# 87003697/DynamiCrafter

Hardware: AMD Instinct MI355X
Metric: frames/sec (and denoising-step ms), 16f@576x1024, DDIM 50 (higher is better)
Workload: dtype bf16; 1 GPU; inference_1024_v1.0.yaml: 1 clip/GPU, 16 frames, latent 72x128, DDIM 50 uniform_trailing eta=1, CFG 7.5 batched (cond+uncond), guidance_rescale 0.7, v-param+ZTSNR+dynamic rescale, hipGraph-captured step; clips_per_gpu=1, parallelism=dp1 over 1 distinct clips (no data-path collective), conditioning=local (1 rank), outputs_finite=True

## Files before the change

### dynamicrafter_amd/_hip.py

```python
import ctypes as C
import os
import threading

_HERE = os.path.dirname(os.path.abspath(__file__))
LIB_PATH = os.environ.get("DC_HIP_LIB") or os.path.join(_HERE, "csrc", "libdcrafter_hip.so")

DC_GEMM_OUT_F32 = 1
DC_GEMM_GEGLU = 2
DC_GEMM_GELU = 4


class DcGemmParams(C.Structure):
    _fields_ = [
        ("A", C.c_void_p), ("W", C.c_void_p), ("C", C.c_void_p), ("bias", C.c_void_p),
        ("rowvec", C.c_void_p), ("residual", C.c_void_p),
        ("lda", C.c_int), ("ldc", C.c_int), ("ldr", C.c_int), ("rowvec_ld", C.c_int),
        ("rows_per_vec", C.c_int),
        ("M", C.c_int), ("N", C.c_int), ("K", C.c_int), ("n_pad", C.c_int),
        ("mode", C.c_int), ("Cin", C.c_int),
        ("IH", C.c_int), ("IW", C.c_int), ("OH", C.c_int), ("OW", C.c_int),
        ("stride", C.c_int), ("pad", C.c_int), ("ups", C.c_int),
        ("T", C.c_int), ("HW", C.c_int),
        ("flags", C.c_int), ("alpha", C.c_float),
        ("workspace", C.c_void_p), ("workspace_bytes", C.c_longlong),
# ... 49 lines not shown
        ("step_index", C.c_void_p), ("index", C.c_int), ("weight_type", C.c_int), ("x0_param", C.c_int),
        ("e_nchw", C.c_int), ("cfg_scale", C.c_float), ("guidance_rescale", C.c_float),
        ("beta2", C.c_float), ("eps", C.c_float), ("one_minus_beta1", C.c_float), ("one_minus_beta2", C.c_float),
        ("decay", C.c_float), ("grad_scale", C.c_float), ("noise_step_stride", C.c_int64), ("loss", C.c_void_p),
    ]


_P, _I, _F, _L = C.c_void_p, C.c_int, C.c_float, C.c_int64
SIGNATURES = {
    "dc_gemm_conv": (_I, [C.POINTER(DcGemmParams), _P]),
    "dc_gemm_workspace_bytes": (_L, []),
    "dc_gemm_last_variant": (C.c_char_p, []),
    "dc_gemm_set_plan": (_I, [_I]),
    "dc_groupnorm": (_I, [_P, _I, _P, _I, _P, _P, _I, _I, _I, _I, _F, _I, _P, _P]),
    "dc_groupnorm_workspace_bytes": (_L, [_I, _I, _I]),
    "dc_layernorm": (_I, [_P, _I, _P, _I, _P, _P, _I, _I, _F, _P]),
    "dc_flash_attn_d64": (_I, [_P, _P, _P, _P, _I, _I, _I, _I, _I, _I, _I, _I, _L, _L, _F, _I, _F, _P]),
    "dc_ff_geglu_fused320": (_I, [_P, _I, _P, _P, _F, _P, _P, _P, _P, _P, _I, _P, _I, _I, _P]),
    "dc_ff_geglu_proj_fused320": (_I, [_P, _I, _P, _P, _F, _P, _P, _P, _P, _P, _P, _P, _I, _P, _I, _I, _P]),
    "dc_ln_linear": (_I, [_P, _I, _I, _P, _P, _F, _P, _P, _P, _I, _I, _I, _P]),
    "dc_ln_qkv_temporal_attn320": (_I, [_P, _I, _P, _P, _F, _P, _P, _I, _I, _I, _I, _F, _P]),
    "dc_ln_qkv_temporal_attn640": (_I, [_P, _I, _P, _P, _F, _P, _P, _I, _I, _I, _I, _F, _P]),
    "dc_gn_silu_tconv3": (_I, [_P, _I, _I, _P, _P, _P, _I, _P, _P, _P, _I, _P, _I, _I, _I, _I, _I, _P]),
    "dc_groupnorm_stats": (_I, [_P, _I, _I, _I, _I, _I, _F, _P, _P, _P]),
    "dc_gn_linear": (_I, [_P, _I, _I, _P, _P, _P, _I, _I, _P, _P, _P, _I, _I, _I, _P]),
    "dc_flash_attn_set_mode": (_I, [_I, _F]),
    "dc_linear_residual": (_I, [_P, _I, _I, _P, _P, _P, _I, _P, _I, _I, _I, _P]),
    "dc_cross_attn_dual_d64": (_I, [_P, _P, _P, _P, _P, _P, _I, _I, _I, _I, _I, _I, _I, _I, _L, _L, _F, _F, _P]),
    "dc_temporal_attn_d64": (_I, [_P, _I, _P, _I, _I, _I, _I, _I, _F, _P]),
    "dc_gemv_small": (_I, [_P, _I, _P, _P, _P, _I, _I, _I, _I, _I, _I, _I, _P]),
    "dc_timestep_embedding": (_I, [_P, _P, _I, _P, _I, _I, _F, _P]),
    "dc_pack_latent": (_I, [_P, _P, _P, _I, _I, _I, _I, _I, _I, _I, _P]),
    "dc_pack_latent_windows": (_I, [_P, _P, _P, _P, _P] + [_I] * 13 + [_P]),
    "dc_window_merge": (_I, [_P, _I, _P, _I, _P, _P, _P] + [_I] * 12 + [_P]),
    "dc_nchw_to_rows": (_I, [_P, _P, _I, _I, _I, _I, _F, _P]),
    "dc_rows_to_nchw": (_I, [_P, _I, _I, _P, _I, _I, _I, _F, _P]),
    "dc_im2col3x3_c8": (_I, [_P, _I, _P, _I, _I, _I, _I, _P]),
    "dc_copy2d": (_I, [_P, _I, _P, _I, _I, _I, _P]),
    "dc_build_context": (_I, [_P, _P, _I, _I, _I, _I, _I, _P]),
    "dc_softmax_rows": (_I, [_P, _I, _P, _I, _I, _I, _P]),
    "dc_transpose": (_I, [_P, _I, _P, _I, _I, _I, _P]),
    "dc_add_rows": (_I, [_P, _I, _P, _I, _P, _I, _I, _I, _P]),
    "dc_vae_sample": (_I, [_P, _I, _P, _P, _I, _I, _I, _F, _P]),
    "dc_ddim_step": (_I, [C.POINTER(DcDdimParams), _P, _P, _P, _I, _P, _P, _P, _P, _I, _I, _I, _P, _P]),
    "dc_ddim_invert_step": (_I, [C.POINTER(DcInvertParams), _P, _P, _P, _I, _P, _P, _P, _I, _I, _I, _P, _P]),
    "dc_dpmpp_step": (_I, [C.POINTER(DcDpmParams), _P, _P, _P, _I, _P, _P, _P, _P, _I, _I, _I, _P, _P]),
# ... 92 lines not shown
```

### dynamicrafter_amd/csrc/dc_common.h

```cpp
#pragma once
#include <hip/hip_runtime.h>
#include <stdint.h>
#include <atomic>

typedef uint16_t bf16_t;

typedef __attribute__((ext_vector_type(8))) short bf16x8_t;
typedef __attribute__((ext_vector_type(4))) short bf16x4_t;
typedef __attribute__((ext_vector_type(16))) float f32x16_t;
typedef __attribute__((ext_vector_type(4))) float f32x4_t;
typedef __attribute__((ext_vector_type(4))) unsigned int u32x4_t;

#define DC_WAVE 64

__device__ __forceinline__ float bf2f(bf16_t v) {
    return __uint_as_float(((uint32_t)v) << 16);
}

typedef __attribute__((ext_vector_type(2))) float f32x2_t;
typedef __attribute__((ext_vector_type(2))) __bf16 bf16x2_hw_t;

__device__ __forceinline__ uint32_t pack_bf2(float lo, float hi) {
    const f32x2_t v = {lo, hi};
    return __builtin_bit_cast(uint32_t, __builtin_convertvector(v, bf16x2_hw_t));
// ... 67 lines not shown
    return v;
}
__device__ __forceinline__ float wave_max(float v) {
#pragma unroll
    for (int o = 32; o > 0; o >>= 1) v = fmaxf(v, __shfl_xor(v, o, 64));
    return v;
}

__device__ __forceinline__ int xcd_remap(int bid, int nwg) {
    const int q = nwg >> 3, r = nwg & 7;
    const int xcd = bid & 7, idx = bid >> 3;
    const int base = (xcd < r) ? xcd * (q + 1) : r * (q + 1) + (xcd - r) * q;
    return base + idx;
}

void dc_note_variant(const char* name);

int dc_gemm_plan_now();

int dc_flash_pipe_launch(const bf16_t* q, const bf16_t* k, const bf16_t* v, bf16_t* o, int ldq, int ldk, int ldv, int ldo,
                         int batch, int heads, int Lq, int Lk, int64_t q_bstride, int64_t kv_bstride, float c,
                         hipStream_t stream);

int* dc_error_word_device();
#define DC_ERRW_GEMM_PIPE 1
#define DC_ERRW_FLASH_RING 2
#define DC_ERRW_GEMM_PP 4

struct DcLdsOnce {
    std::atomic<unsigned long long> done{0};
    int ensure(const void* fn, int bytes) {
        int dev = 0;
        hipError_t e = hipGetDevice(&dev);
        if (e != hipSuccess) return (int)e;
        const bool tracked = dev >= 0 && dev < 64;
        if (tracked && (done.load(std::memory_order_acquire) >> dev & 1ull)) return 0;
        e = hipFuncSetAttribute(fn, hipFuncAttributeMaxDynamicSharedMemorySize, bytes);
        if (e != hipSuccess) return (int)e;
        if (tracked) done.fetch_or(1ull << dev, std::memory_order_release);
        return 0;
    }
};

#define DC_CHECK_LAUNCH() do { hipError_t e__ = hipGetLastError(); if (e__ != hipSuccess) return (int)e__; } while (0)
```

### dynamicrafter_amd/csrc/ff_fused.hip

```cpp
#include "attn_parts.h"
#include "dc_common.h"
#include "dcrafter_hip.h"
#include "lds_stage.h"
#include <stdint.h>
#include <type_traits>

namespace {

constexpr int FD = 320;
constexpr int FM = 4 * FD;
constexpr int FCH = 32;
constexpr int FNCH = FM / FCH;
constexpr int FBM = 128;
constexpr int W1_STAGE = 64 * FD * 2;
constexpr int W2_STAGE = FD * FCH * 2;
constexpr int W2_RING = 3;
constexpr int FF_LDS = 2 * W1_STAGE + W2_RING * W2_STAGE + 4 * 2048 + 2 * FM * 4;
static_assert(FF_LDS <= 160 * 1024, "LDS");

#ifdef DC_FF_STAMPS
__device__ unsigned long long g_ff_stamps[8];
#define FF_STAMP(i) do { asm volatile("s_waitcnt lgkmcnt(0)" ::: "memory"); const unsigned long long t__ = __builtin_readcyclecounter(); \
                         st_acc[i] += t__ - st_last; st_last = t__; } while (0)
#else
// ... 833 lines not shown
        {
            const int rrow = lane >> 3, rc = lane & 7;
#pragma unroll
            for (int t = 0; t < 4; ++t) {
                const int r = t * 8 + rrow;
                const u32x4_t d = *reinterpret_cast<const u32x4_t*>(vpatch + lds_off128(r, rc));
                *reinterpret_cast<u32x4_t*>(p.O + grow(r) * p.ldo + 64 * h + rc * 8) = d;
            }
        }
    }
}


struct TcParams {
    const bf16_t* X; int ldx;
    const bf16_t* W;
    const float* bias;
    const bf16_t* R; int ldr;
    bf16_t* O; int ldo;
    const float* gn_g; const float* gn_b; const float2* gn_stats; int gn_groups;
    int HW, N;
    int nsplit, cpp;
    int ntiles;
};

template <int KH, bool RES>
__global__ __launch_bounds__(256, 2)
void gn_silu_tconv_kernel(const TcParams p) {
    constexpr int KD = FD * KH;
    extern __shared__ __attribute__((aligned(16))) char smem[];
    const int tid = threadIdx.x;
    const int lane = tid & 63;
    const int wave = __builtin_amdgcn_readfirstlane(tid >> 6);
    const int fr = lane & 31, fh = lane >> 5;
    const unsigned lds_base = (unsigned)(unsigned long)((lds_char_t*)smem);
    char* const ebuf = smem + 2 * LW_STAGE + wave * 2048;
    float* const lns = reinterpret_cast<float*>(smem + 2 * LW_STAGE + 4 * 2048);
    float* const bls = lns + 2 * KD;
    const bool bias_lds = KH == 1 && p.N <= LL_BIAS;
    const XsPart part = xs_part_decode(p.nsplit, p.cpp, p.N / LCH);
    const int tile = part.tile, c_begin = part.c_begin, c_end = part.c_end;
    if (tile >= p.ntiles) return;
    const int gpb = p.HW >> 3;
    const int b = tile / gpb, p0 = (tile - b * gpb) * 8 + 2 * wave;
    const XsRowsGather grow{b, p.HW, p0};
    if (c_begin >= c_end) return;

    unsigned vo[5];
    xs_piece_offsets<3 * KD * 2, 384>(vo, wave, lane);
    auto w_base = [&](int c, int j) {
        const int jt = j / KH, h = j - jt * KH;
        const int tap = jt == 0 ? 1 : (jt == 1 ? 0 : 2);
        return (uint64_t)(uintptr_t)p.W + (uint64_t)c * (LCH * 3 * KD * 2) + tap * 128 + h * (5 * 384);
    };
    xs_issue_stage(lds_base, 0, wave, vo, w_base(c_begin, 0));

    bf16x8_t xf[KD / 16];
    xs_load_rows(xf, p.X + grow(fr) * p.ldx + fh * 8);
    xs_stage_gn_affine(lns, KD, p.gn_g, p.gn_b, p.gn_stats + (size_t)b * p.gn_groups, p.gn_groups, tid);
    if (bias_lds) xs_stage_bias(bls, p.bias, p.N, tid);
    asm volatile("s_waitcnt vmcnt(0) lgkmcnt(0)" ::: "memory");
    __builtin_amdgcn_s_barrier();
    asm volatile("" ::: "memory");
    affine_rows_inplace<KD, true>(xf, lns, lns + KD, fh);

    constexpr int PD = KH == 1 ? 6 : 3;
    constexpr int NS = 3 * KH;
    int slot = 0;
    for (int c = c_begin; c < c_end; ++c) {
        f32x16_t out, y;
        u32x4_t rres[2];
#pragma unroll
        for (int j = 0; j < NS; ++j) {
            const int jt = j / KH, h = j % KH;
            if (c > c_begin || j > 0) {
                if (j == 0) { if (RES && KH != 1) wait_vmcnt<4>(); else wait_vmcnt<2>(); }
                else wait_vmcnt<0>();
                __builtin_amdgcn_s_barrier();
                asm volatile("" ::: "memory");
            }
            if constexpr (RES && KH == 1) {
                if (j == 0) {
#pragma unroll
                    for (int t = 0; t < 2; ++t)
                        rres[t] = *reinterpret_cast<const u32x4_t*>(p.R + grow(t * 16 + (lane >> 2)) * p.ldr + c * LCH + (lane & 3) * 8);
                }
            }
            f32x16_t& acc = jt == 0 ? out : y;
            if (h == 0) {
#pragma unroll
                for (int r = 0; r < 16; ++r) acc[r] = 0.f;
            }
            const bool more = j + 1 < NS || c + 1 < c_end;
            const uint64_t nb = j + 1 < NS ? w_base(c, j + 1) : w_base(c + 1, 0);
            xs_stage_mma<PD>(smem + slot * LW_STAGE, xf, h * (FD / 16), acc, fr, fh, [&](int i) __attribute__((always_inline)) {
                if (more) lds_dma16_sbase(xs_stage_dst(lds_base, (slot ^ 1) * LW_STAGE, wave, i), vo[i], nb);
            });
            slot ^= 1;
            if (jt > 0 && h == KH - 1) {
#pragma unroll
                for (int r = 0; r < 16; ++r) {
                    const float yv = y[r];
                    out[r] += __int_as_float(jt == 1 ? __builtin_amdgcn_update_dpp(0, __float_as_int(yv), 0x111, 0xf, 0xf, false)
                                                     : __builtin_amdgcn_update_dpp(0, __float_as_int(yv), 0x101, 0xf, 0xf, false));
                }
            }
        }
        {
            const int n0 = c * LCH;
            const int rrow = lane >> 2, rc = lane & 3;
            if constexpr (RES) {
                if constexpr (KH != 1) {
#pragma unroll
                    for (int t = 0; t < 2; ++t) rres[t] = *reinterpret_cast<const u32x4_t*>(p.R + grow(t * 16 + rrow) * p.ldr + n0 + rc * 8);
                }
#pragma unroll
                for (int t = 0; t < 2; ++t) *xs_patch_row(ebuf, t * 16 + rrow, rc) = rres[t];
            }
#pragma unroll
            for (int q = 0; q < 4; ++q) {
                float4 bv = bias_lds ? *reinterpret_cast<const float4*>(bls + n0 + 8 * q + 4 * fh)
                                     : *reinterpret_cast<const float4*>(p.bias + n0 + 8 * q + 4 * fh);
                uint2* const slot2 = xs_patch_acc(ebuf, fr, fh, q);
                if constexpr (RES) xs_add_bf16x4(bv, *slot2);
                *slot2 = xs_pack_acc(out, q, bv);
            }
#pragma unroll
            for (int t = 0; t < 2; ++t) {
                const int r = t * 16 + rrow;
                const u32x4_t d = *xs_patch_row(ebuf, r, rc);
                *reinterpret_cast<u32x4_t*>(p.O + grow(r) * p.ldo + n0 + rc * 8) = d;
            }
        }
    }
}

}

#ifdef DC_FF_STAMPS
extern "C" int dc_ff_debug_stamps(unsigned long long* out, int reset) {
    hipError_t e = hipMemcpyFromSymbol(out, HIP_SYMBOL(g_ff_stamps), sizeof(unsigned long long) * 8);
    if (e == hipSuccess && reset) {
        unsigned long long z[8] = {0};
        e = hipMemcpyToSymbol(HIP_SYMBOL(g_ff_stamps), z, sizeof(z));
    }
    return (int)e;
}
#endif

template <bool LN, bool PROJ>
static int launch_ff_fused(const FfParams& p, hipStream_t stream) {
    static DcLdsOnce lds_once;
    if (const int e = lds_once.ensure(reinterpret_cast<const void*>(&ff_geglu_fused320_kernel<LN, PROJ>), FF_LDS)) return e;
    const int tiles = (p.M + FBM - 1) / FBM;
    hipLaunchKernelGGL((ff_geglu_fused320_kernel<LN, PROJ>), dim3(tiles < 256 ? tiles : 256), dim3(256), FF_LDS, stream, p);
// ... 118 lines not shown
    if (const int e = lds_once.ensure(reinterpret_cast<const void*>(&ln_qkv_tattn_kernel<KH>), ta_lds(KH))) return e;
    TaParams p;
    p.X = x; p.ldx = ldx; p.W = wqkv; p.O = out; p.ldo = ldo; p.ln_g = ln_gamma; p.ln_b = ln_beta; p.ln_eps = ln_eps;
    p.HW = HW; p.c = scale * 1.4426950408889634f;
    static const int hsplit_env = [] { const char* e = getenv("DC_TA_HSPLIT"); return e ? atoi(e) : 0; }();
    const int hsplit = (KH == 2 && hsplit_env == 2) ? 2 : 1;
    hipLaunchKernelGGL(ln_qkv_tattn_kernel<KH>, dim3((unsigned)(B * (HW / 8)), hsplit), dim3(256), ta_lds(KH), (hipStream_t)stream_, p);
    DC_CHECK_LAUNCH();
    return 0;
}

extern "C" int dc_ln_qkv_temporal_attn320(const uint16_t* x, int ldx, const float* ln_gamma, const float* ln_beta, float ln_eps,
                                          const uint16_t* wqkv, uint16_t* out, int ldo, int B, int T, int HW, float scale,
                                          void* stream_) {
    return launch_ln_qkv_tattn<1>(x, ldx, ln_gamma, ln_beta, ln_eps, wqkv, out, ldo, B, T, HW, scale, stream_);
}

extern "C" int dc_ln_qkv_temporal_attn640(const uint16_t* x, int ldx, const float* ln_gamma, const float* ln_beta, float ln_eps,
                                          const uint16_t* wqkv, uint16_t* out, int ldo, int B, int T, int HW, float scale,
                                          void* stream_) {
    return launch_ln_qkv_tattn<2>(x, ldx, ln_gamma, ln_beta, ln_eps, wqkv, out, ldo, B, T, HW, scale, stream_);
}

template <int KH, bool RES>
static int launch_gn_silu_tconv(const TcParams& p, dim3 grid, hipStream_t stream) {
    static DcLdsOnce lds_once;
    if (const int e = lds_once.ensure(reinterpret_cast<const void*>(&gn_silu_tconv_kernel<KH, RES>), ll_lds(KH))) return e;
    hipLaunchKernelGGL((gn_silu_tconv_kernel<KH, RES>), grid, dim3(256), ll_lds(KH), stream, p);
    DC_CHECK_LAUNCH();
    return 0;
}

extern "C" int dc_gn_silu_tconv3(const uint16_t* x, int ldx, int C, const float* gamma, const float* beta, const float* stats,
                                 int groups, const uint16_t* w, const float* bias, const uint16_t* residual, int ldr,
                                 uint16_t* out, int ldo, int B, int T, int HW, int N, void* stream_) {
    if (!x || !gamma || !beta || !stats || !w || !bias || !out) return DC_ERR_ARG;
    if ((C != FD && C != 2 * FD) || B < 1 || T != 16 || HW < 8 || HW % 8 || N < LCH || N % LCH || ldx % 8 || ldo % 8 ||
        (residual && ldr % 8)) return DC_ERR_SHAPE;
    if (groups < 1 || C % groups) return DC_ERR_SHAPE;
    if (((uintptr_t)x | (uintptr_t)out | (uintptr_t)w | (uintptr_t)(residual ? residual : out)) % 16) return DC_ERR_SHAPE;
    TcParams p;
    p.X = x; p.ldx = ldx; p.W = w; p.bias = bias; p.R = residual; p.ldr = ldr; p.O = out; p.ldo = ldo;
    p.gn_g = gamma; p.gn_b = beta; p.gn_stats = reinterpret_cast<const float2*>(stats); p.gn_groups = groups; p.HW = HW; p.N = N;
    p.ntiles = B * (HW / 8);
    const XsSplit sp = xs_split_n(p.ntiles, N / LCH, 256 * 2);
    p.nsplit = sp.nsplit; p.cpp = sp.cpp;
    const dim3 grid = sp.grid;
    hipStream_t stream = (hipStream_t)stream_;
    if (C == FD) return residual ? launch_gn_silu_tconv<1, true>(p, grid, stream) : launch_gn_silu_tconv<1, false>(p, grid, stream);
    return residual ? launch_gn_silu_tconv<2, true>(p, grid, stream) : launch_gn_silu_tconv<2, false>(p, grid, stream);
}
```

### dynamicrafter_amd/csrc/norms.hip

```cpp
#include "dc_common.h"
#include "dcrafter_hip.h"
#include <stdlib.h>

namespace {

struct GnGeom { int chunks; int rows_per_chunk; };

__host__ __device__ inline GnGeom gn_geom(int n_inst, int rows_per_inst) {
    int chunks = (2048 + n_inst - 1) / n_inst;
    int rpc = (rows_per_inst + chunks - 1) / chunks;
    if (rpc < 64) rpc = 64;
    GnGeom g;
    g.rows_per_chunk = rpc;
    g.chunks = (rows_per_inst + rpc - 1) / rpc;
    return g;
}

__global__ void gn_partial_kernel(const bf16_t* __restrict__ x, int ldx, int C, int groups, int rows_per_inst,
                                  int rows_per_chunk, int chunks, int vecs, int rpp, float2* __restrict__ partial) {
    extern __shared__ float sm[];
    const int inst = blockIdx.y, chunk = blockIdx.x;
    const int v = threadIdx.x % vecs;
    const int ro = threadIdx.x / vecs;
    const int r_begin = chunk * rows_per_chunk;
// ... 43 lines not shown
        for (int rr = 0; rr < rpp; ++rr) {
            const int first = r_begin + rr;
            const float nb = first < r_end ? (float)((r_end - first + rpp - 1) / rpp) : 0.f;
            if (nb == 0.f) continue;
            for (int c = 0; c < cpg; ++c) {
                const float mb = sm_s[rr * C + g * cpg + c], qb = sm_q[rr * C + g * cpg + c];
                const float nn = n + nb;
                const float w = nb * __builtin_amdgcn_rcpf(nn);
                const float delta = mb - mean;
                mean += delta * w;
                m2 += qb + delta * delta * (n * w);
                n = nn;
            }
        }
        partial[((size_t)inst * chunks + chunk) * groups + g] = make_float2(mean, m2);
    }
}

__global__ __launch_bounds__(64) void gn_finalize_kernel(const float2* __restrict__ partial, int chunks, int groups,
                                                         int rows_per_inst, int rows_per_chunk, int cpg, float eps,
                                                         float2* __restrict__ stats) {
    const int g = blockIdx.x, inst = blockIdx.y;
    float n = 0.f, mean = 0.f, m2 = 0.f;
    for (int c = threadIdx.x; c < chunks; c += 64) {
        const float2 p = partial[((size_t)inst * chunks + c) * groups + g];
        int rows = rows_per_inst - c * rows_per_chunk;
        if (rows > rows_per_chunk) rows = rows_per_chunk;
        const float nb = (float)rows * (float)cpg;
        const float nn = n + nb;
        const float w = nb * __builtin_amdgcn_rcpf(nn);
        const float delta = p.x - mean;
        mean += delta * w;
        m2 += p.y + delta * delta * (n * w);
        n = nn;
    }
#pragma unroll
    for (int o = 32; o > 0; o >>= 1) {
        const float nb = __shfl_xor(n, o, 64), mb = __shfl_xor(mean, o, 64), qb = __shfl_xor(m2, o, 64);
        const float nn = n + nb;
        if (nn > 0.f) {
            const float w = nb * __builtin_amdgcn_rcpf(nn);
            const float delta = mb - mean;
            mean += delta * w;
            m2 += qb + delta * delta * (n * w);
            n = nn;
        }
    }
    if (threadIdx.x == 0) {
        float var = m2 / n;
        if (var < 0.f) var = 0.f;
        stats[(size_t)inst * groups + g] = make_float2(mean, rsqrtf(var + eps));
    }
}

template <bool FIN>
__global__ void gn_apply_kernel(const bf16_t* __restrict__ x, int ldx, bf16_t* __restrict__ y, int ldy,
                                const float* __restrict__ gamma, const float* __restrict__ beta, int C, int groups,
// ... 198 lines not shown
                                  float* workspace, float* stats_out, void* stream_) {
    hipStream_t stream = (hipStream_t)stream_;
    if (!x || !workspace || !stats_out) return DC_ERR_ARG;
    if (C % 8 != 0 || groups <= 0 || groups > 64 || C % groups != 0 || ldx % 8 != 0) return DC_ERR_SHAPE;
    if (n_inst <= 0 || rows_per_inst <= 0) return DC_ERR_SHAPE;
    const int vecs = C / 8;
    if (vecs > 1024) return DC_ERR_SHAPE;
    int rpp = 256 / vecs;
    if (rpp < 1) rpp = 1;
    const int threads = vecs * rpp;
    const GnGeom g = gn_geom(n_inst, rows_per_inst);
    float2* partial = reinterpret_cast<float2*>(workspace);
    const size_t lds = (size_t)2 * rpp * C * sizeof(float);
    if (lds > 64 * 1024) return DC_ERR_SHAPE;
    hipLaunchKernelGGL(gn_partial_kernel, dim3(g.chunks, n_inst), dim3(threads), lds, stream, x, ldx, C, groups,
                       rows_per_inst, g.rows_per_chunk, g.chunks, vecs, rpp, partial);
    DC_CHECK_LAUNCH();
    hipLaunchKernelGGL(gn_finalize_kernel, dim3(groups, n_inst), dim3(64), 0, stream, partial, g.chunks, groups, rows_per_inst,
                       g.rows_per_chunk, C / groups, eps, reinterpret_cast<float2*>(stats_out));
    DC_CHECK_LAUNCH();
    return 0;
}

extern "C" int dc_layernorm(const uint16_t* x, int ldx, uint16_t* y, int ldy, const float* gamma, const float* beta,
                            int rows, int C, float eps, void* stream_) {
    hipStream_t stream = (hipStream_t)stream_;
    if (!x || !y || !gamma || !beta) return DC_ERR_ARG;
    if (C % 8 != 0 || C > 2048 || ldx % 8 != 0 || ldy % 8 != 0 || rows <= 0) return DC_ERR_SHAPE;
    int grid = (rows + 7) / 8;
    if (grid > 8192) grid = 8192;
    const int vecs = C / 8;
    if (vecs <= 64)
        hipLaunchKernelGGL(layernorm_kernel<1>, dim3(grid), dim3(256), 0, stream, x, ldx, y, ldy, gamma, beta, rows, C, eps);
    else if (vecs <= 128)
        hipLaunchKernelGGL(layernorm_kernel<2>, dim3(grid), dim3(256), 0, stream, x, ldx, y, ldy, gamma, beta, rows, C, eps);
    else
        hipLaunchKernelGGL(layernorm_kernel<4>, dim3(grid), dim3(256), 0, stream, x, ldx, y, ldy, gamma, beta, rows, C, eps);
    DC_CHECK_LAUNCH();
    return 0;
}
```

### dynamicrafter_amd/lvdm/modules/networks/openaimodel3d.py

```python
import math

import torch
import torch.nn as nn

from .... import ops
from ....ops import PackedWeight
from ....param_tree import attach_params

import os

_BF16 = torch.bfloat16
_FF_FUSED = os.environ.get("DC_FF_FUSED", "1") != "0"
_LN_FUSED = os.environ.get("DC_LN_FUSED", "1") != "0"
_LR_FUSED = os.environ.get("DC_LR_FUSED", "1") != "0"
_TA_FUSED = os.environ.get("DC_TA_FUSED", "1") != "0"
_TA_FUSED_C = tuple(int(k) for k in os.environ.get("DC_TA_FUSED_C", "320,640").split(","))
_FFP_FUSED = os.environ.get("DC_FFP_FUSED", "1") != "0"
_TC_FUSED = os.environ.get("DC_TC_FUSED", "1") != "0"
_FUSED_MIN_ROWS = int(os.environ.get("DC_FUSED_MIN_ROWS", "4096"))
_LN_FUSED_K = tuple(int(k) for k in os.environ.get("DC_LN_FUSED_K", "320,640").split(","))
C_IN_PAD = 64


def _block_layout(cfg):
    mc, mults, nrb = cfg["model_channels"], list(cfg["channel_mult"]), cfg["num_res_blocks"]
    attn_res = set(cfg["attention_resolutions"])
    hc = cfg["num_head_channels"]
    tconv = bool(cfg["temporal_conv"])

    def transformers(ch):
        out = [("spatial", {"ch": ch, "heads": ch // hc})]
        if cfg["temporal_attention"]:
            out.append(("temporal", {"ch": ch, "inner": ch, "heads": ch // hc, "linear": bool(cfg["use_linear"])}))
        return out

    down_path = [[("conv_in", {"cin": cfg["in_channels"], "cout": mc})]]
    widths = [mc]
    ch, ds = mc, 1
    for lvl, m in enumerate(mults):
        for _ in range(nrb):
            blk = [("res", {"cin": ch, "cout": m * mc, "tconv": tconv})]
# ... 356 lines not shown
        ops.gemv_small(g["emb"], W["emb"], emb_out, act_in=1)
        h = self._gn(x, W["gn1"], "gn", n_inst=g["F"], rpi=g["HW"], eps=1e-5, silu=True)
        h1 = ops.gemm(h, W["conv1"], A.get("res_h1", M, cout, device=dev), conv=conv, rowvec=emb_out,
                      rows_per_vec=g["T"] * g["HW"])
        h = self._gn(h1, W["gn2"], "gn", n_inst=g["F"], rpi=g["HW"], eps=1e-5, silu=True)
        skip = x
        if "skip" in W:
            skip = ops.gemm(x, W["skip"], A.get("res_skip", M, cout, device=dev))
        has_tc = "tc" in W
        final = (lambda: out if out is not None else A.get(out_tag, M, cout, device=dev))
        h2 = ops.gemm(h, W["conv2"], A.get("res_h2", M, cout, device=dev) if has_tc else final(), conv=conv,
                      residual=skip)
        if not has_tc:
            return h2
        tc = dict(T=g["T"], HW=g["HW"])
        r = h2
        fused_tc = (_TC_FUSED and cout in _LN_FUSED_K and g["T"] == 16 and g["HW"] % 8 == 0 and M >= _FUSED_MIN_ROWS
                    and (g["T"] * g["HW"]) % 128 == 0)
        for i, (gnw, cw) in enumerate(W["tc"]):
            last = i == 3
            dst = final() if last else A.get("res_ta" if i % 2 == 0 else "res_tb", M, cout, device=dev)
            if fused_tc:
                st = A.get("gn_stats", g["B"] * 32 * 2, 1, torch.float32, dev)
                ops.groupnorm_stats(r, st, groups=32, n_inst=g["B"], rows_per_inst=g["T"] * g["HW"], eps=1e-5)
                r = ops.gn_silu_tconv3(r, gnw[0], gnw[1], st, cw, dst, B=g["B"], T=16, HW=g["HW"],
                                           residual=h2 if last else None)
                continue
            n = self._gn(r, gnw, "gn", n_inst=g["B"], rpi=g["T"] * g["HW"], eps=1e-5, silu=True)
            r = ops.gemm(n, cw, dst, tconv=tc, residual=h2 if last else None)
        return r

    def _ln_linear(self, h, ln, pw, out):
        if _LN_FUSED and pw.K in _LN_FUSED_K and pw.N % 32 == 0 and h.shape[0] >= _FUSED_MIN_ROWS:
            return ops.ln_linear(h, pw, out, ln=ln, ln_eps=1e-5)
        return ops.gemm(self._ln(h, ln, "ln"), pw, out)

    def _lin_res(self, x, pw, res, out):
        if _LR_FUSED and pw.K in _LN_FUSED_K and pw.N % 32 == 0 and x.shape[0] >= _FUSED_MIN_ROWS:
            return ops.linear_residual(x, pw, res, out)
        return ops.gemm(x, pw, out, residual=res)

    def _gn_linear(self, x, gnw, pw, out, *, n_inst, rpi):
        if _LN_FUSED and pw.K in _LN_FUSED_K and pw.N % 32 == 0 and x.shape[0] >= _FUSED_MIN_ROWS and rpi % 128 == 0:
            st = self._arena.get("gn_stats", n_inst * 32 * 2, 1, torch.float32, x.device)
            ops.groupnorm_stats(x, st, groups=32, n_inst=n_inst, rows_per_inst=rpi, eps=1e-6)
            return ops.gn_linear(x, gnw[0], gnw[1], st, pw, out, groups=32, rows_per_inst=rpi)
        return ops.gemm(self._gn(x, gnw, "gn", n_inst=n_inst, rpi=rpi, eps=1e-6, silu=False), pw, out)

# ... 281 lines not shown
```

### dynamicrafter_amd/ops.py

```python
import ctypes as C
import os
import math

import torch

from . import _hip
from ._hip import DcDdimParams, DcGemmParams, check

_BF16 = torch.bfloat16


def stream_ptr():
    return C.c_void_p(torch.cuda.current_stream().cuda_stream)


class Tracer:

    def __init__(self):
        self.records = []

    def __enter__(self):
        global _TRACE
        _TRACE = self
        return self
# ... 408 lines not shown
    _need_rows(x, M, K, "x"); _need_rows(out, M, pw.N, "out"); _need_rows(residual, M, pw.N, "residual")
    _launch("linear_residual", 2.0 * M * pw.N * K, 2.0 * M * (K + 2 * pw.N) + 2.0 * pw.N * K, _hip.lib().dc_linear_residual,
            _ptr(x), x.stride(0), K, _ptr(pw.w), _ptr(pw.bias), _ptr(residual), residual.stride(0), _ptr(out), out.stride(0),
            M, pw.N, stream_ptr())
    return out


def ln_qkv_temporal_attn(x, ln, pw_qkv, out, *, B, T, HW, scale, ln_eps=1e-5):
    _rows(x, "x"); _rows(out, "out")
    M = B * T * HW
    Cc = pw_qkv.K
    if Cc not in (320, 640) or pw_qkv.N != 3 * Cc or pw_qkv.bias is not None or T != 16 or HW % 8:
        raise ValueError("ln_qkv_temporal_attn: dim 320 / 640 (qkv weight [3 C, C], no bias), T = 16, HW % 8 == 0")
    if x.data_ptr() == out.data_ptr():
        raise ValueError("ln_qkv_temporal_attn: out must not alias x")
    _need_rows(x, M, Cc, "x"); _need_rows(out, M, Cc, "out"); _need(ln[0], Cc, "ln gamma"); _need(ln[1], Cc, "ln beta")
    fn = _hip.lib().dc_ln_qkv_temporal_attn320 if Cc == 320 else _hip.lib().dc_ln_qkv_temporal_attn640
    _launch(f"ln_qkv_temporal_attn{Cc}", 2.0 * M * 3 * Cc * Cc + 4.0 * M * T * Cc, 4.0 * M * Cc + 2.0 * 3 * Cc * Cc,
            fn, _ptr(x), x.stride(0), _ptr(ln[0]), _ptr(ln[1]), ln_eps, _ptr(pw_qkv.w),
            _ptr(out), out.stride(0), B, T, HW, scale, stream_ptr())
    return out


def gn_silu_tconv3(x, gamma, beta, stats, pw, out, *, B, T, HW, groups=32, residual=None):
    _rows(x, "x"); _rows(out, "out")
    M = B * T * HW
    C = pw.w.shape[1] // 3
    if C not in (320, 640) or pw.w.shape[1] != 3 * C or pw.N % 32 or pw.bias is None or T != 16 or HW % 8:
        raise ValueError("gn_silu_tconv3: 320 / 640 input channels (weight [N, 3 C] with bias), N % 32 == 0, T = 16, HW % 8 == 0")
    if x.data_ptr() == out.data_ptr():
        raise ValueError("gn_silu_tconv3: out must not alias x")
    _need_rows(x, M, C, "x"); _need_rows(out, M, pw.N, "out")
    _need(gamma, C, "gamma"); _need(beta, C, "beta"); _need(stats, B * groups * 2, "stats")
    if residual is not None:
        _rows(residual, "residual"); _need_rows(residual, M, pw.N, "residual")
    _launch("gn_silu_tconv3", 2.0 * M * pw.N * 3 * C, 2.0 * M * (C + pw.N * (2 if residual is not None else 1)) + 2.0 * pw.N * 3 * C,
            _hip.lib().dc_gn_silu_tconv3, _ptr(x), x.stride(0), C, _ptr(gamma), _ptr(beta), _ptr(stats), groups, _ptr(pw.w),
            _ptr(pw.bias), _ptr(residual), 0 if residual is None else residual.stride(0), _ptr(out), out.stride(0), B, T, HW,
            pw.N, stream_ptr())
    return out


def groupnorm_stats(x, stats, *, groups, n_inst, rows_per_inst, eps):
    _rows(x, "x")
    Cc = x.shape[1]
    _need_rows(x, n_inst * rows_per_inst, Cc, "x"); _need(stats, n_inst * groups * 2, "stats")
    l = _hip.lib()
    ws = _gn_workspace(x.device, int(l.dc_groupnorm_workspace_bytes(n_inst, groups, rows_per_inst)))
    _launch("groupnorm_stats(2 kernels)", 0.0, 2.0 * n_inst * rows_per_inst * Cc, l.dc_groupnorm_stats, _ptr(x), x.stride(0),
            Cc, groups, n_inst, rows_per_inst, eps, _ptr(ws), _ptr(stats), stream_ptr())
    return stats


def gn_linear(x, gamma, beta, stats, pw, out, *, groups, rows_per_inst):
    _rows(x, "x"); _rows(out, "out")
    M, K = x.shape[0], pw.K
    if K not in (320, 640) or pw.N % 32 or rows_per_inst % 128 or M % rows_per_inst:
        raise ValueError("gn_linear: K in (320, 640), N % 32 == 0, rows_per_inst % 128 == 0, M % rows_per_inst == 0")
# ... 1037 lines not shown
```

### include/dcrafter_hip.h

```cpp
#ifndef DCRAFTER_HIP_H
#define DCRAFTER_HIP_H
#include <stdint.h>

#ifdef __cplusplus
extern "C" {
#endif

#define DC_ERR_SHAPE (-1)
#define DC_ERR_ARG   (-2)

#define DC_GEMM_OUT_F32 1
#define DC_GEMM_GEGLU   2
#define DC_GEMM_GELU    4

typedef struct DcGemmParams {
    const uint16_t* A;
    const uint16_t* W;
    void* C;
    const float* bias;
    const float* rowvec;
    const uint16_t* residual;
    int lda, ldc, ldr, rowvec_ld;
    int rows_per_vec;
    int M, N, K, n_pad;
// ... 176 lines not shown

int dc_ff_geglu_proj_fused320(const uint16_t* x, int ldx, const float* ln_gamma, const float* ln_beta, float ln_eps,
                              const uint16_t* w1, const float* b1, const uint16_t* w2p, const float* b2, const uint16_t* wp,
                              const float* bp, const uint16_t* residual2, int ldr2, uint16_t* out, int ldo, int M, void* stream);

int dc_ln_linear(const uint16_t* x, int ldx, int K, const float* ln_gamma, const float* ln_beta, float ln_eps, const uint16_t* w,
                 const float* bias, uint16_t* out, int ldo, int M, int N, void* stream);
int dc_groupnorm_stats(const uint16_t* x, int ldx, int C, int groups, int n_inst, int rows_per_inst, float eps,
                       float* workspace, float* stats_out, void* stream);
int dc_gn_linear(const uint16_t* x, int ldx, int K, const float* gamma, const float* beta, const float* stats, int groups,
                 int rows_per_inst, const uint16_t* w, const float* bias, uint16_t* out, int ldo, int M, int N, void* stream);

int dc_linear_residual(const uint16_t* x, int ldx, int K, const uint16_t* w, const float* bias, const uint16_t* residual, int ldr,
                       uint16_t* out, int ldo, int M, int N, void* stream);

int dc_ln_qkv_temporal_attn320(const uint16_t* x, int ldx, const float* ln_gamma, const float* ln_beta, float ln_eps,
                               const uint16_t* wqkv, uint16_t* out, int ldo, int B, int T, int HW, float scale, void* stream);
int dc_ln_qkv_temporal_attn640(const uint16_t* x, int ldx, const float* ln_gamma, const float* ln_beta, float ln_eps,
                               const uint16_t* wqkv, uint16_t* out, int ldo, int B, int T, int HW, float scale, void* stream);

int dc_gn_silu_tconv3(const uint16_t* x, int ldx, int C, const float* gamma, const float* beta, const float* stats, int groups,
                      const uint16_t* w, const float* bias, const uint16_t* residual, int ldr, uint16_t* out, int ldo, int B, int T,
                      int HW, int N, void* stream);


int dc_attn_small(const uint16_t* q, const uint16_t* k, const uint16_t* v, uint16_t* o, int ldq, int ldk, int ldv, int ldo,
                  int B, int heads, int Lq, int Lk, int d, float scale, int causal, void* stream);
int64_t dc_attn_small_lds_bytes(int Lk, int d);

int dc_clip_preprocess(const float* img, float* tmp0, float* tmp1, float* out, int N, int C, int H, int W, int OH, int OW,
                       int antialias, const float* mean3, const float* std3, void* stream);

int dc_patchify(const float* img, uint16_t* rows, int N, int C, int H, int W, int p, int kpad, void* stream);

int dc_embed_tokens(const int64_t* tokens, const uint16_t* table, const uint16_t* pos, uint16_t* out, int B, int L, int D,
                    int vocab, void* stream);

int dc_frames_to_u8(const float* video, uint8_t* out, int N, int C, int T, int H, int W, void* stream);


#define DC_JPEG_MCU_MAX_BYTES 2496

int dc_jpeg_dct_quant(const uint8_t* frames, const uint8_t* qtab, int16_t* coef, int T, int H, int W, void* stream);

int dc_jpeg_entropy(const int16_t* coef, uint8_t* scratch, int32_t* seg_len, int T, int my, int mx, int ri, int64_t stride,
                    void* stream);
// ... 131 lines not shown
```

Before: 2.645 frames/s.

## Fuse next-stage GroupNorm statistics into GN-SiLU temporal conv epilogue

Measured after the change: 2.659 frames/s, median of 6. No clear change (+0.5%).

```diff
diff --git a/dynamicrafter_amd/_hip.py b/dynamicrafter_amd/_hip.py
--- a/dynamicrafter_amd/_hip.py
+++ b/dynamicrafter_amd/_hip.py
@@ -95,6 +95,7 @@
     "dc_ln_qkv_temporal_attn320": (_I, [_P, _I, _P, _P, _F, _P, _P, _I, _I, _I, _I, _F, _P]),
     "dc_ln_qkv_temporal_attn640": (_I, [_P, _I, _P, _P, _F, _P, _P, _I, _I, _I, _I, _F, _P]),
     "dc_gn_silu_tconv3": (_I, [_P, _I, _I, _P, _P, _P, _I, _P, _P, _P, _I, _P, _I, _I, _I, _I, _I, _P]),
+    "dc_gn_silu_tconv3_stats": (_I, [_P, _I, _I, _P, _P, _P, _I, _P, _P, _P, _I, _I, _I, _I, _I, _F, _P, _P, _P]),
     "dc_groupnorm_stats": (_I, [_P, _I, _I, _I, _I, _I, _F, _P, _P, _P]),
     "dc_gn_linear": (_I, [_P, _I, _I, _P, _P, _P, _I, _I, _P, _P, _P, _I, _I, _I, _P]),
     "dc_flash_attn_set_mode": (_I, [_I, _F]),
diff --git a/dynamicrafter_amd/csrc/dc_common.h b/dynamicrafter_amd/csrc/dc_common.h
--- a/dynamicrafter_amd/csrc/dc_common.h
+++ b/dynamicrafter_amd/csrc/dc_common.h
@@ -113,6 +113,9 @@
                          int batch, int heads, int Lq, int Lk, int64_t q_bstride, int64_t kv_bstride, float c,
                          hipStream_t stream);
 
+int dc_gn_finalize_launch(const float* partial, int chunks, int groups, int n_inst, int rows_per_inst, int rows_per_chunk, int cpg,
+                          float eps, float* stats_out, hipStream_t stream);
+
 int* dc_error_word_device();
 #define DC_ERRW_GEMM_PIPE 1
 #define DC_ERRW_FLASH_RING 2
diff --git a/dynamicrafter_amd/csrc/ff_fused.hip b/dynamicrafter_amd/csrc/ff_fused.hip
--- a/dynamicrafter_amd/csrc/ff_fused.hip
+++ b/dynamicrafter_amd/csrc/ff_fused.hip
@@ -879,11 +879,54 @@
     int HW, N;
     int nsplit, cpp;
     int ntiles;
+    float2* partial; int groups_out;
 };
 
-template <int KH, bool RES>
+__device__ __forceinline__ int xs_patch_tr_off(int lane) {
+    const int r = 8 * (lane >> 4) + ((lane & 15) >> 2), s = lane & 3;
+    return r * 64 + ((s ^ (((r >> 1) & 3) << 1)) << 3);
+}
+
+struct TcStats {
+    unsigned a0, a1;
+    int dsel;
+    bool diag_lane;
+    float2* row;
+    bf16x4_t tq[4];
+    __device__ __forceinline__ void init(unsigned patch, int lane, float2* wave_row) {
+        const unsigned off = (unsigned)xs_patch_tr_off(lane);
+        a0 = patch + off; a1 = patch + (off ^ 32);
+        dsel = lane & 3; diag_lane = (lane >> 4) == ((lane & 15) >> 2);
+        row = wave_row + (lane & 15);
+    }
+    __device__ __forceinline__ void issue() {
+        asm volatile("ds_read_b64_tr_b16 %0, %4\n\tds_read_b64_tr_b16 %1, %5 offset:256\n\t"
+                     "ds_read_b64_tr_b16 %2, %5\n\tds_read_b64_tr_b16 %3, %4 offset:256"
+                     : "=&v"(tq[0]), "=&v"(tq[1]), "=&v"(tq[2]), "=&v"(tq[3]) : "v"(a0), "v"(a1) : "memory");
+    }
+    __device__ __forceinline__ void finish(int n0) {
+        asm volatile("s_waitcnt lgkmcnt(0)" : "+v"(tq[0]), "+v"(tq[1]), "+v"(tq[2]), "+v"(tq[3]) :: "memory");
+        const short one = 0x3f80;
+        const bf16x8_t ones = {one, one, one, one, one, one, one, one};
+        const f32x4_t zero = {0.f, 0.f, 0.f, 0.f};
+#pragma unroll
+        for (int cb = 0; cb < 2; ++cb) {
+            const bf16x8_t pf = attn_vt_join(tq[2 * cb], tq[2 * cb + 1]);
+            const f32x4_t sv = __builtin_amdgcn_mfma_f32_16x16x32_bf16(ones, pf, zero, 0, 0, 0);
+            const f32x4_t qv = __builtin_amdgcn_mfma_f32_16x16x32_bf16(pf, pf, zero, 0, 0, 0);
+            float sq = qv[0];
+#pragma unroll
+            for (int r = 1; r < 4; ++r) sq = dsel == r ? qv[r] : sq;
+            const float mean = sv[0] * (1.0f / 32);
+            if (diag_lane) row[n0 + 16 * cb] = make_float2(mean, fmaxf(sq - sv[0] * mean, 0.f));
+        }
+    }
+};
+
+template <int KH, bool RES, bool STATS = false>
 __global__ __launch_bounds__(256, 2)
 void gn_silu_tconv_kernel(const TcParams p) {
+    static_assert(!(RES && STATS), "the last stage's consumer is a per-frame norm");
     constexpr int KD = FD * KH;
     extern __shared__ __attribute__((aligned(16))) char smem[];
     const int tid = threadIdx.x;
@@ -923,6 +966,9 @@
 
     constexpr int PD = KH == 1 ? 6 : 3;
     constexpr int NS = 3 * KH;
+    float2* const gtab = reinterpret_cast<float2*>(smem + ll_lds(KH));
+    [[maybe_unused]] TcStats ts;
+    if constexpr (STATS && KH == 1) ts.init(lds_base + 2 * LW_STAGE + wave * 2048, lane, gtab + wave * p.N);
     int slot = 0;
     for (int c = c_begin; c < c_end; ++c) {
         f32x16_t out, y;
@@ -950,9 +996,11 @@
             }
             const bool more = j + 1 < NS || c + 1 < c_end;
             const uint64_t nb = j + 1 < NS ? w_base(c, j + 1) : w_base(c + 1, 0);
+            if constexpr (STATS && KH == 1) { if (j == 0 && c > c_begin) ts.issue(); }
             xs_stage_mma<PD>(smem + slot * LW_STAGE, xf, h * (FD / 16), acc, fr, fh, [&](int i) __attribute__((always_inline)) {
                 if (more) lds_dma16_sbase(xs_stage_dst(lds_base, (slot ^ 1) * LW_STAGE, wave, i), vo[i], nb);
             });
+            if constexpr (STATS && KH == 1) { if (j == 0 && c > c_begin) ts.finish((c - 1) * LCH); }
             slot ^= 1;
             if (jt > 0 && h == KH - 1) {
 #pragma unroll
@@ -988,6 +1036,41 @@
                 const u32x4_t d = *xs_patch_row(ebuf, r, rc);
                 *reinterpret_cast<u32x4_t*>(p.O + grow(r) * p.ldo + n0 + rc * 8) = d;
             }
+            if constexpr (STATS && KH != 1) {
+                int l = lane;
+                asm volatile("" : "+v"(l));
+                ts.init(lds_base + 2 * LW_STAGE + wave * 2048, l, gtab + wave * p.N);
+                ts.issue();
+                ts.finish(n0);
+            }
+        }
+    }
+    if constexpr (STATS) {
+        const int cpg = p.N / p.groups_out;
+        const int g0 = c_begin * LCH / cpg, ng = (c_end - c_begin) * LCH / cpg;
+        float2* const wtab = gtab + 4 * p.N;
+        auto chan = [](float& n, float& mean, float& m2, float nb, float2 t) __attribute__((always_inline)) {
+            const float nn = n + nb;
+            const float wgt = nb * __builtin_amdgcn_rcpf(nn);
+            const float delta = t.x - mean;
+            mean += delta * wgt;
+            m2 += t.y + delta * delta * (n * wgt);
+            n = nn;
+        };
+        if constexpr (KH == 1) { ts.issue(); ts.finish((c_end - 1) * LCH); }
+        __builtin_amdgcn_wave_barrier();
+        if (lane < ng) {
+            float n = 0.f, mean = 0.f, m2 = 0.f;
+            const float2* const row = gtab + wave * p.N + (g0 + lane) * cpg;
+            for (int cc = 0; cc < cpg; ++cc) chan(n, mean, m2, 32.f, row[cc]);
+            wtab[wave * 64 + lane] = make_float2(mean, m2);
+        }
+        __syncthreads();
+        if (tid < ng) {
+            float n = 0.f, mean = 0.f, m2 = 0.f;
+#pragma unroll
+            for (int w = 0; w < 4; ++w) chan(n, mean, m2, 32.f * (float)cpg, wtab[w * 64 + tid]);
+            p.partial[(size_t)tile * p.groups_out + g0 + tid] = make_float2(mean, m2);
         }
     }
 }
@@ -1152,12 +1235,28 @@
     return launch_ln_qkv_tattn<2>(x, ldx, ln_gamma, ln_beta, ln_eps, wqkv, out, ldo, B, T, HW, scale, stream_);
 }
 
-template <int KH, bool RES>
+template <int KH, bool RES, bool STATS = false>
 static int launch_gn_silu_tconv(const TcParams& p, dim3 grid, hipStream_t stream) {
     static DcLdsOnce lds_once;
-    if (const int e = lds_once.ensure(reinterpret_cast<const void*>(&gn_silu_tconv_kernel<KH, RES>), ll_lds(KH))) return e;
-    hipLaunchKernelGGL((gn_silu_tconv_kernel<KH, RES>), grid, dim3(256), ll_lds(KH), stream, p);
+    constexpr int lds_max = ll_lds(KH) + (STATS ? 4 * (LL_BIAS + 64) * 8 : 0);
+    static_assert(2 * lds_max <= 160 * 1024, "LDS");
+    if (const int e = lds_once.ensure(reinterpret_cast<const void*>(&gn_silu_tconv_kernel<KH, RES, STATS>), lds_max)) return e;
+    hipLaunchKernelGGL((gn_silu_tconv_kernel<KH, RES, STATS>), grid, dim3(256), ll_lds(KH) + (STATS ? 4 * (p.N + 64) * 8 : 0), stream, p);
     DC_CHECK_LAUNCH();
+    return 0;
+}
+
+static int tc_params(TcParams& p, const uint16_t* x, int ldx, int C, const float* gamma, const float* beta, const float* stats,
+                     int groups, const uint16_t* w, const float* bias, const uint16_t* residual, int ldr, uint16_t* out, int ldo,
+                     int B, int T, int HW, int N) {
+    if ((C != FD && C != 2 * FD) || B < 1 || T != 16 || HW < 8 || HW % 8 || N < LCH || N % LCH || ldx % 8 || ldo % 8 ||
+        (residual && ldr % 8)) return DC_ERR_SHAPE;
+    if (groups < 1 || C % groups) return DC_ERR_SHAPE;
+    if (((uintptr_t)x | (uintptr_t)out | (uintptr_t)w | (uintptr_t)(residual ? residual : out)) % 16) return DC_ERR_SHAPE;
+    p.X = x; p.ldx = ldx; p.W = w; p.bias = bias; p.R = residual; p.ldr = ldr; p.O = out; p.ldo = ldo;
+    p.gn_g = gamma; p.gn_b = beta; p.gn_stats = reinterpret_cast<const float2*>(stats); p.gn_groups = groups; p.HW = HW; p.N = N;
+    p.ntiles = B * (HW / 8);
+    p.partial = nullptr; p.groups_out = groups;
     return 0;
 }
 
@@ -1165,14 +1264,8 @@
                                  int groups, const uint16_t* w, const float* bias, const uint16_t* residual, int ldr,
                                  uint16_t* out, int ldo, int B, int T, int HW, int N, void* stream_) {
     if (!x || !gamma || !beta || !stats || !w || !bias || !out) return DC_ERR_ARG;
-    if ((C != FD && C != 2 * FD) || B < 1 || T != 16 || HW < 8 || HW % 8 || N < LCH || N % LCH || ldx % 8 || ldo % 8 ||
-        (residual && ldr % 8)) return DC_ERR_SHAPE;
-    if (groups < 1 || C % groups) return DC_ERR_SHAPE;
-    if (((uintptr_t)x | (uintptr_t)out | (uintptr_t)w | (uintptr_t)(residual ? residual : out)) % 16) return DC_ERR_SHAPE;
     TcParams p;
-    p.X = x; p.ldx = ldx; p.W = w; p.bias = bias; p.R = residual; p.ldr = ldr; p.O = out; p.ldo = ldo;
-    p.gn_g = gamma; p.gn_b = beta; p.gn_stats = reinterpret_cast<const float2*>(stats); p.gn_groups = groups; p.HW = HW; p.N = N;
-    p.ntiles = B * (HW / 8);
+    if (const int e = tc_params(p, x, ldx, C, gamma, beta, stats, groups, w, bias, residual, ldr, out, ldo, B, T, HW, N)) return e;
     const XsSplit sp = xs_split_n(p.ntiles, N / LCH, 256 * 2);
     p.nsplit = sp.nsplit; p.cpp = sp.cpp;
     const dim3 grid = sp.grid;
@@ -1180,3 +1273,20 @@
     if (C == FD) return residual ? launch_gn_silu_tconv<1, true>(p, grid, stream) : launch_gn_silu_tconv<1, false>(p, grid, stream);
     return residual ? launch_gn_silu_tconv<2, true>(p, grid, stream) : launch_gn_silu_tconv<2, false>(p, grid, stream);
 }
+
+extern "C" int dc_gn_silu_tconv3_stats(const uint16_t* x, int ldx, int C, const float* gamma, const float* beta, const float* stats,
+                                       int groups, const uint16_t* w, const float* bias, uint16_t* out, int ldo, int B, int T,
+                                       int HW, int N, float eps_next, float* partial_out, float* stats_out, void* stream_) {
+    if (!x || !gamma || !beta || !stats || !w || !bias || !out || !partial_out || !stats_out) return DC_ERR_ARG;
+    TcParams p;
+    if (const int e = tc_params(p, x, ldx, C, gamma, beta, stats, groups, w, bias, nullptr, 0, out, ldo, B, T, HW, N)) return e;
+    if (N > LL_BIAS || N % groups || groups > 64) return DC_ERR_SHAPE;
+    const XsSplit sp = xs_split_n(p.ntiles, N / LCH, 256 * 2);
+    p.nsplit = sp.nsplit; p.cpp = sp.cpp;
+    if (sp.nsplit > 1 && ((N / LCH) % sp.nsplit || (sp.cpp * LCH) % (N / groups))) return DC_ERR_SHAPE;
+    p.partial = reinterpret_cast<float2*>(partial_out);
+    hipStream_t stream = (hipStream_t)stream_;
+    if (const int e = C == FD ? launch_gn_silu_tconv<1, false, true>(p, sp.grid, stream)
+                              : launch_gn_silu_tconv<2, false, true>(p, sp.grid, stream)) return e;
+    return dc_gn_finalize_launch(partial_out, HW / 8, groups, B, 16 * HW, FBM, N / groups, eps_next, stats_out, stream);
+}
diff --git a/dynamicrafter_amd/csrc/norms.hip b/dynamicrafter_amd/csrc/norms.hip
--- a/dynamicrafter_amd/csrc/norms.hip
+++ b/dynamicrafter_amd/csrc/norms.hip
@@ -89,17 +89,29 @@
                                                          float2* __restrict__ stats) {
     const int g = blockIdx.x, inst = blockIdx.y;
     float n = 0.f, mean = 0.f, m2 = 0.f;
-    for (int c = threadIdx.x; c < chunks; c += 64) {
-        const float2 p = partial[((size_t)inst * chunks + c) * groups + g];
-        int rows = rows_per_inst - c * rows_per_chunk;
-        if (rows > rows_per_chunk) rows = rows_per_chunk;
-        const float nb = (float)rows * (float)cpg;
-        const float nn = n + nb;
-        const float w = nb * __builtin_amdgcn_rcpf(nn);
-        const float delta = p.x - mean;
-        mean += delta * w;
-        m2 += p.y + delta * delta * (n * w);
-        n = nn;
+    constexpr int U = 8;
+    for (int c0 = threadIdx.x; c0 < chunks; c0 += 64 * U) {
+        float2 pv[U];
+#pragma unroll
+        for (int u = 0; u < U; ++u) {
+            const int c = c0 + 64 * u;
+            pv[u] = partial[((size_t)inst * chunks + (c < chunks ? c : c0)) * groups + g];
+        }
+#pragma unroll
+        for (int u = 0; u < U; ++u) {
+            const int c = c0 + 64 * u;
+            if (c >= chunks) break;
+            const float2 p = pv[u];
+            int rows = rows_per_inst - c * rows_per_chunk;
+            if (rows > rows_per_chunk) rows = rows_per_chunk;
+            const float nb = (float)rows * (float)cpg;
+            const float nn = n + nb;
+            const float w = nb * __builtin_amdgcn_rcpf(nn);
+            const float delta = p.x - mean;
+            mean += delta * w;
+            m2 += p.y + delta * delta * (n * w);
+            n = nn;
+        }
     }
 #pragma unroll
     for (int o = 32; o > 0; o >>= 1) {
@@ -344,6 +356,14 @@
     return 0;
 }
 
+int dc_gn_finalize_launch(const float* partial, int chunks, int groups, int n_inst, int rows_per_inst, int rows_per_chunk, int cpg,
+                          float eps, float* stats_out, hipStream_t stream) {
+    hipLaunchKernelGGL(gn_finalize_kernel, dim3(groups, n_inst), dim3(64), 0, stream, reinterpret_cast<const float2*>(partial), chunks,
+                       groups, rows_per_inst, rows_per_chunk, cpg, eps, reinterpret_cast<float2*>(stats_out));
+    DC_CHECK_LAUNCH();
+    return 0;
+}
+
 extern "C" int dc_layernorm(const uint16_t* x, int ldx, uint16_t* y, int ldy, const float* gamma, const float* beta,
                             int rows, int C, float eps, void* stream_) {
     hipStream_t stream = (hipStream_t)stream_;
diff --git a/dynamicrafter_amd/lvdm/modules/networks/openaimodel3d.py b/dynamicrafter_amd/lvdm/modules/networks/openaimodel3d.py
--- a/dynamicrafter_amd/lvdm/modules/networks/openaimodel3d.py
+++ b/dynamicrafter_amd/lvdm/modules/networks/openaimodel3d.py
@@ -17,6 +17,8 @@
 _TA_FUSED_C = tuple(int(k) for k in os.environ.get("DC_TA_FUSED_C", "320,640").split(","))
 _FFP_FUSED = os.environ.get("DC_FFP_FUSED", "1") != "0"
 _TC_FUSED = os.environ.get("DC_TC_FUSED", "1") != "0"
+_TC_STATS = os.environ.get("DC_TC_STATS", "1") != "0"
+_TC_STATS_C = tuple(int(k) for k in os.environ.get("DC_TC_STATS_C", "320,640").split(","))
 _FUSED_MIN_ROWS = int(os.environ.get("DC_FUSED_MIN_ROWS", "4096"))
 _LN_FUSED_K = tuple(int(k) for k in os.environ.get("DC_LN_FUSED_K", "320,640").split(","))
 C_IN_PAD = 64
@@ -419,8 +421,15 @@
             dst = final() if last else A.get("res_ta" if i % 2 == 0 else "res_tb", M, cout, device=dev)
             if fused_tc:
                 st = A.get("gn_stats", g["B"] * 32 * 2, 1, torch.float32, dev)
-                ops.groupnorm_stats(r, st, groups=32, n_inst=g["B"], rows_per_inst=g["T"] * g["HW"], eps=1e-5)
-                r = ops.gn_silu_tconv3(r, gnw[0], gnw[1], st, cw, dst, B=g["B"], T=16, HW=g["HW"],
+                tc_stats = _TC_STATS and cout in _TC_STATS_C
+                if i == 0 or not tc_stats:
+                    ops.groupnorm_stats(r, st, groups=32, n_inst=g["B"], rows_per_inst=g["T"] * g["HW"], eps=1e-5)
+                if tc_stats and not last:
+                    part = A.get("gn_partial_tc", g["B"] * (g["HW"] // 8) * 32 * 2, 1, torch.float32, dev)
+                    r = ops.gn_silu_tconv3(r, gnw[0], gnw[1], st, cw, dst, B=g["B"], T=16, HW=g["HW"], stats_out=st,
+                                           partial_out=part, eps_next=1e-5)
+                else:
+                    r = ops.gn_silu_tconv3(r, gnw[0], gnw[1], st, cw, dst, B=g["B"], T=16, HW=g["HW"],
                                            residual=h2 if last else None)
                 continue
             n = self._gn(r, gnw, "gn", n_inst=g["B"], rpi=g["T"] * g["HW"], eps=1e-5, silu=True)
diff --git a/dynamicrafter_amd/ops.py b/dynamicrafter_amd/ops.py
--- a/dynamicrafter_amd/ops.py
+++ b/dynamicrafter_amd/ops.py
@@ -454,7 +454,8 @@
     return out
 
 
-def gn_silu_tconv3(x, gamma, beta, stats, pw, out, *, B, T, HW, groups=32, residual=None):
+def gn_silu_tconv3(x, gamma, beta, stats, pw, out, *, B, T, HW, groups=32, residual=None, stats_out=None, partial_out=None,
+                   eps_next=1e-5):
     _rows(x, "x"); _rows(out, "out")
     M = B * T * HW
     C = pw.w.shape[1] // 3
@@ -466,6 +467,16 @@
     _need(gamma, C, "gamma"); _need(beta, C, "beta"); _need(stats, B * groups * 2, "stats")
     if residual is not None:
         _rows(residual, "residual"); _need_rows(residual, M, pw.N, "residual")
+    if stats_out is not None:
+        if residual is not None or partial_out is None:
+            raise ValueError("gn_silu_tconv3: stats_out needs partial_out and takes no residual")
+        n_part = B * (HW // 8) * groups * 2
+        _need(stats_out, B * groups * 2, "stats_out"); _need(partial_out, n_part, "partial_out")
+        _launch("gn_silu_tconv3", 2.0 * M * pw.N * 3 * C, 2.0 * M * (C + pw.N) + 2.0 * pw.N * 3 * C + 8.0 * n_part,
+                _hip.lib().dc_gn_silu_tconv3_stats, _ptr(x), x.stride(0), C, _ptr(gamma), _ptr(beta), _ptr(stats), groups,
+                _ptr(pw.w), _ptr(pw.bias), _ptr(out), out.stride(0), B, T, HW, pw.N, eps_next, _ptr(partial_out),
+                _ptr(stats_out), stream_ptr())
+        return out
     _launch("gn_silu_tconv3", 2.0 * M * pw.N * 3 * C, 2.0 * M * (C + pw.N * (2 if residual is not None else 1)) + 2.0 * pw.N * 3 * C,
             _hip.lib().dc_gn_silu_tconv3, _ptr(x), x.stride(0), C, _ptr(gamma), _ptr(beta), _ptr(stats), groups, _ptr(pw.w),
             _ptr(pw.bias), _ptr(residual), 0 if residual is None else residual.stride(0), _ptr(out), out.stride(0), B, T, HW,
diff --git a/include/dcrafter_hip.h b/include/dcrafter_hip.h
--- a/include/dcrafter_hip.h
+++ b/include/dcrafter_hip.h
@@ -222,6 +222,9 @@
 int dc_gn_silu_tconv3(const uint16_t* x, int ldx, int C, const float* gamma, const float* beta, const float* stats, int groups,
                       const uint16_t* w, const float* bias, const uint16_t* residual, int ldr, uint16_t* out, int ldo, int B, int T,
                       int HW, int N, void* stream);
+int dc_gn_silu_tconv3_stats(const uint16_t* x, int ldx, int C, const float* gamma, const float* beta, const float* stats,
+                            int groups, const uint16_t* w, const float* bias, uint16_t* out, int ldo, int B, int T, int HW, int N,
+                            float eps_next, float* partial_out, float* stats_out, void* stream);
 
 
 int dc_attn_small(const uint16_t* q, const uint16_t* k, const uint16_t* v, uint16_t* o, int ldq, int ldk, int ldv, int ldo,
```
